# AER-RC/monoRTM

Hardware: AMD Instinct MI355X
Metric: (wavenumber x layer x line) optical-depth evals/sec (higher is better)
Workload: dtype f64; 1 GPU; c4: configs[3] whole: 1024 synthetic sonde profiles x 64 layers x 50 channels x 500 lines, f64, profile-sharded over 1 GPU(s): 1024 profiles on this rank; layers=64, wavenumbers=50, lines=500, nmol=7, launch=3 stream launches, parallelism=profile-sharded x1

## Files before the change

monortm_amd/_build.py:

```python
from __future__ import annotations

import os
import shutil
import subprocess

PKG = os.path.dirname(os.path.abspath(__file__))
ROOT = os.path.dirname(PKG)
CSRC = os.path.join(PKG, "csrc")
FSRC = os.path.join(PKG, "fortran")
LIBDIR = os.path.join(PKG, "lib")
LIB = os.path.join(LIBDIR, "libmonortm_hip.so")

HIPCC = os.environ.get("HIPCC", "/opt/rocm/bin/hipcc")
FC = os.environ.get("MONORTM_FC", "/opt/rocm/bin/amdflang")
HIP_SOURCES = ["api.hip", "lines_kernel.hip", "lines_ms_kernel.hip", "far_kernel.hip", "continuum_kernel.hip", "xsec_kernel.hip", "xsec_jac_kernel.hip", "rtm_kernel.hip", "rtm_scan_kernel.hip", "jacobian_kernel.hip", "rtm_scan_jac_kernel.hip", "rtm_obs_jac_kernel.hip", "rtm_obs_kernel.hip", "oe_kernel.hip", "line_table.cpp"]
HIP_DEPS = HIP_SOURCES + ["device_common.hpp", "lineshape.hpp", "cloud_tkc.hpp", "obs_exchange.hpp", "rtm_tile.hpp", "modm_plan.hpp", "ms_reach.hpp", "lines_device.hpp", "xsec_walk.hpp", "lines_asm.hpp", "lines_ms_asm.hpp", "line_table.hpp", "tables/monortm_tables.h",
                           "../../include/monortm_hip.h"]
HIP_FLAGS = ["--offload-arch=gfx950", "-O3", "-std=c++17", "-fPIC", "-shared", "-Wno-unused-value", "-Wno-pass-failed",
             "-Wno-unused-const-variable"]


_NO_LICM = ["-mllvm", "-disable-machine-licm"]
HIP_FILE_FLAGS = {"lines_ms_kernel.hip": _NO_LICM, "lines_kernel.hip": _NO_LICM, "continuum_kernel.hip": _NO_LICM, "rtm_obs_kernel.hip": _NO_LICM}


def _check_flags(flags: list[str]) -> None:
    extra = os.environ.get("MONORTM_EXTRA_HIPFLAGS", "").split()
    bad = [f for f in flags + extra if f.startswith(("-DFAR_ABL_", "-DMONORTM_ABLATE_", "-DMONORTM_NO_", "-DLINES_TIMING", "-DLINES_CLASS_STATS",
                                                     "-DMW_TIMING"))]
    if bad and os.environ.get("MONORTM_EXPERIMENT") != "1":
        raise RuntimeError(f"experiment switches in the build flags {bad}: set MONORTM_EXPERIMENT=1 (and use tools/build_variant.sh)")
# ... 82 lines not shown
```

monortm_amd/csrc/api.hip:

```cpp
#include <algorithm>
#include <atomic>
#include <chrono>
#include <cmath>
#include <cstdlib>
#include <cstdio>
#include <cstring>
#include <dlfcn.h>
#include <functional>
#include <initializer_list>
#include <string>
#include <vector>

#include "device_common.hpp"
#include "line_table.hpp"
#include "modm_plan.hpp"
#include "lineshape.hpp"
#include "tables/monortm_tables.h"

namespace {
using namespace monortm_dev;

thread_local std::string g_init_error;

struct Ctx {
    int device = 0;
    int cus = 256;
    size_t phys_cap = 2ull << 30, far_cap = 1ull << 30;
    std::vector<Ctx *> shards;
    struct Opt : ModmPlanOpt {
        int ms_ablate = 0;
        int ms_prepare = MS_PREPARE_FUSED;
        int ms_plan = 1;
        double jac_dt = MONORTM_JAC_DT, jac_dlnw = MONORTM_JAC_DLNW;
    } opt;
    void *comm = nullptr;
    int comm_rank = 0, comm_world = 1;
    bool has_lines = false;
    int real_kind = 8;
    std::string err;
    monortm::LineTable host;
    DevLines lines{};
    DevTables tables{};
    std::vector<void *> owned;
    int *errflag = nullptr;
    void *partial = nullptr;
    monortm_dev::MwCache mw_cache;
    void *phys = nullptr;
// ... 38 lines not shown
        const double *wpath = nullptr, *mw = nullptr;
        std::vector<int> shard;
    };
    static constexpr int kMaxObs = 16;
    Obs obs[kMaxObs];
    hipStream_t hs = nullptr;
    int *errflag_host = nullptr;
    struct {
        const void *dev = nullptr, *host = nullptr;
        size_t bytes = 0;
        int nprof = 0, nwn = 0, nlay_max = 0;
    } lastO;
    long long o_reused = 0;
    long long o_reused_scan = 0;
    long long finish_launches[6] = {0, 0, 0, 0, 0, 0};
    long long far_launches[4] = {0, 0, 0, 0};
    bool host_timing = false;
    double ht[3][4] = {{0, 0, 0, 0}, {0, 0, 0, 0}, {0, 0, 0, 0}};
    long long ht_calls[3] = {0, 0, 0};
    size_t partial_elems = 0;
    int profiling = 0;
    int prof_stride = 1;
    long long prof_calls[3] = {0, 0, 0};
    struct Ev {
        hipEvent_t a, b;
        int k;
    };
    std::vector<Ev> events;
    std::vector<hipEvent_t> event_pool;
    double tot_ms[3] = {0, 0, 0};
// ... 27 lines not shown
                           static_cast<const uint4 *>(src2), static_cast<uint4 *>(dst2), bytes2 / 16, flag_src, flag_dst);
        return hipGetLastError();
    }
    hipError_t e = hipMemcpyAsync(dst, src, bytes, kind, s);
    if (e == hipSuccess && flag_dst) e = hipMemcpyAsync(flag_dst, flag_src, sizeof(int), hipMemcpyDeviceToHost, s);
    if (e == hipSuccess && bytes2) e = hipMemcpyAsync(dst2, src2, bytes2, hipMemcpyDefault, s);
    return e;
}

void comm_release(Ctx *c);

int set_option(Ctx *c, const char *name, const char *value) {
    const std::string n = name ? name : "", v = value ? value : "";
    const bool autov = v.empty() || v == "auto";
    long iv = 0;
    double dv = 0.;
    bool isint = false, isdbl = false;
    if (!autov) {
        char *end = nullptr;
        iv = strtol(v.c_str(), &end, 10);
        isint = end && end != v.c_str() && *end == '\0';
        end = nullptr;
        dv = strtod(v.c_str(), &end);
        isdbl = end && end != v.c_str() && *end == '\0';
    }
    if (n == "nslice" && (autov || (isint && iv >= 1 && iv <= 16))) c->opt.nslice = autov ? 0 : (int)iv;
    else if (n == "fair" && (autov || (isint && (iv == 0 || iv == 1)))) c->opt.fair = autov ? -1 : (int)iv;
    else if (n == "tile_waves" && (autov || (isint && (iv == 1 || iv == 2 || iv == 4)))) c->opt.tile_waves = autov ? 0 : (int)iv;
    else if (n == "far_levels" && (autov || (isint && iv >= 0 && iv <= FAR_MAXLEV))) c->opt.far_levels = autov ? -1 : (int)iv;
    else if (n == "lines_kernel" && (autov || v == "wn" || v == "ms")) c->opt.lines_ms = autov ? -1 : (v == "ms" ? 1 : 0);
    else if (n == "ms_prepare" && (autov || v == "fused" || v == "passes")) c->opt.ms_prepare = v == "passes" ? MS_PREPARE_PASSES : MS_PREPARE_FUSED;
    else if (n == "ms_plan" && (autov || v == "on" || v == "off")) c->opt.ms_plan = v == "off" ? 0 : 1;
#ifdef MONORTM_EXPERIMENT
    else if (n == "ms_ablate" && isint && iv >= 0 && iv <= 9) c->opt.ms_ablate = (int)iv;
#endif
    else if (n == "finish" && (autov || v == "generic")) c->opt.finish_generic = autov ? 0 : 1;
    else if (n == "ms_items" && (autov || (isint && (iv == 64 || iv == 128 || iv == 192 || iv == 256)))) c->opt.ms_items = autov ? 0 : (int)iv;
    else if ((n == "jac_dt" || n == "jac_dlnw") && (autov || (isdbl && std::isfinite(dv) && dv > 0. && (n == "jac_dt" || dv < 1.)))) {
        if (n == "jac_dt") c->opt.jac_dt = autov ? MONORTM_JAC_DT : dv;
        else c->opt.jac_dlnw = autov ? MONORTM_JAC_DLNW : dv;
    }
    else { c->err = "unknown option or value: " + n + " = " + v; return MONORTM_EARG; }
    return MONORTM_OK;
}

template <class T>
int upload(Ctx *c, const T *src, size_t n, const T **dst) {
    void *p = nullptr;
    const size_t bytes = std::max<size_t>(n, 1) * sizeof(T);
    HIPCHK(c, hipMalloc(&p, bytes));
    c->owned.push_back(p);
// ... 802 lines not shown
        }
        if (hipGetLastError() != hipSuccess || hipDeviceSynchronize() != hipSuccess) { c->err = "log-ratio tables could not be formed"; return failed(MONORTM_EHIP); }
    }
    void *ef = nullptr;
    if (hipMalloc(&ef, sizeof(int)) != hipSuccess || hipMemset(ef, 0, sizeof(int)) != hipSuccess) { c->err = "hipMalloc(errflag) failed"; return failed(MONORTM_EHIP); }
    c->owned.push_back(ef);
    c->errflag = static_cast<int *>(ef);
    if (hipDeviceSynchronize() != hipSuccess) { c->err = "device set-up failed"; return failed(MONORTM_EHIP); }
    if (hipStreamCreateWithFlags(&c->hs, hipStreamNonBlocking) != hipSuccess ||
        hipHostMalloc(reinterpret_cast<void **>(&c->errflag_host), sizeof(int), hipHostMallocDefault) != hipSuccess) {
        c->err = "stream / pinned flag of the host-buffer entry points could not be created";
        return failed(MONORTM_EHIP);
    }
    if (const char *e = getenv("MONORTM_HOST_TIMING")) c->host_timing = e[0] == '1';
    if (getenv("MONORTM_FINISH_GENERIC")) c->opt.finish_generic = 1;
    for (const char *k : {"lines_kernel", "nslice", "fair", "tile_waves", "far_levels", "ms_items", "ms_prepare", "ms_plan",
#ifdef MONORTM_EXPERIMENT
                          "ms_ablate",
#endif
                         }) {
        std::string env = "MONORTM_" + std::string(k);
        for (char &ch : env) ch = (char)toupper((unsigned char)ch);
        if (const char *e = getenv(env.c_str()))
            if (set_option(c, k, e)) { c->err = env + ": " + c->err; return failed(MONORTM_EARG); }
    }
    if (c->host_timing && !g_timing_ctx) {
        g_timing_ctx = c;
        static bool registered = false;
        if (!registered) { atexit([] { if (g_timing_ctx) print_host_timing(g_timing_ctx); }); registered = true; }
    }
    *out = c;
// ... 252 lines not shown
    hipFree(din); hipFree(dtab); hipFree(dout);
    return rc ? rc : monortm_hip_check(c, nullptr);
}

long long monortm_hip_counter(void *ctx, int which) {
    Ctx *c = static_cast<Ctx *>(ctx);
    if (!c) return -1;
    if (!c->shards.empty()) {
        long long t = 0;
        for (Ctx *sh : c->shards) t += monortm_hip_counter(sh, which);
        return t;
    }
    if (which == 0) return c->o_reused;
    if (which == 1) return c->o_reused_scan;
    if (which >= 2 && which <= 7) return c->finish_launches[which - 2];
    if (which >= 16 && which <= 19) return c->far_launches[which - 16];
    return -1;
}

long long monortm_hip_line_count(void *ctx, int mol) {
    Ctx *c = static_cast<Ctx *>(ctx);
    if (!c || mol < 0 || mol > MXMOL) return -1;
    if (!c->shards.empty()) c = c->shards[0];
    return c->host.n_physical[mol];
}

int monortm_hip_profile(void *ctx, int enable) {
    Ctx *c = static_cast<Ctx *>(ctx);
    if (!c) return null_ctx();
    if (!c->shards.empty()) return multi_only_host(c);
// ... 184 lines not shown
        aw.nlay = a.nlay + pl.ms_nprof;
        aw.O = const_cast<void *>(shift(a.O, st * nwn)); aw.O_CLW = const_cast<void *>(shift(a.O_CLW, st * nwn));
        aw.O_BY_MOL = const_cast<void *>(shift(a.O_BY_MOL, st * nmol * nwn));
        aw.OC = const_cast<void *>(shift(a.OC, st * MONORTM_NCONT * nwn));
        aw.osum = a.osum ? a.osum + st * nwn : nullptr;
        launch_lines_ms(am, c->lines, c->tables, ms, pl.use_brd, s);
        launch_lines(aw, c->lines, c->tables, pl.nw, pl.wpl, pl.use_brd, dim3(grid.x, (unsigned)aw.nprof, grid.z), pl.dyn_lds, s);
    } else if (pl.use_ms) launch_lines_ms(a, c->lines, c->tables, ms, pl.use_brd, s);
    else launch_lines(a, c->lines, c->tables, pl.nw, pl.wpl, pl.use_brd, grid, pl.dyn_lds, s);
    prof_end(c, s, ev);
    HIPCHK(c, hipGetLastError());
    prof_begin(c, s, 1, ev);
    if (ixsect == 1 && !odx_given) launch_xsec(a, c->xs, s);
    a.slices_reduced = pl.slices_reduced;
    if (pl.slices_reduced) launch_reduce_slices(a, s);
    if (pl.mw) {
        const hipError_t e = launch_finish_mw(a, c->tables, vends[0], vends[1], pl.V1ABS, pl.V2ABS, pl.NPTABS, c->mw_cache, s);
        if (e != hipSuccess) {
            c->err = std::string("launch_finish_mw: ") + (c->mw_cache.why ? c->mw_cache.why : hipGetErrorString(e));
            return c->mw_cache.why ? MONORTM_EUNSUPPORTED : MONORTM_EHIP;
        }
    } else HIPCHK(c, launch_finish(a, c->tables, pl.V1ABS, pl.V2ABS, pl.NPTABS, pl.csize, pl.high, pl.par, pl.fin_threads, pl.fin_lds, pl.lds_sets, s));
    c->finish_launches[pl.finish_variant]++;
    prof_end(c, s, ev);
    HIPCHK(c, hipGetLastError());
    return MONORTM_OK;
}
}

extern "C" {

int monortm_hip_modm_xs_dev(void *ctx, int nprof, int nwn, const double *wn, double dvset, const int *nlay, int nlay_max,
                            int nmol, const void *P, const void *T, const void *CLW, const void *WKL,
                            const void *WBRODL, const double *cntnm_fac, double sclcpl, double sclhw, double y0res,
                            int ibrd, int ixsect, const void *XAMNT, void *ODXSEC, void *O, void *O_BY_MOL, void *OC,
                            void *O_CLW, const double *wn_ends, void *stream) {
    Ctx *c = static_cast<Ctx *>(ctx);
    if (!c) return null_ctx();
// ... 1168 lines not shown
```

monortm_amd/csrc/continuum_kernel.hip:

```cpp
#include "lineshape.hpp"
#include <cstring>
#include "cloud_tkc.hpp"
#include "tables/monortm_tables.h"

namespace {
using namespace monortm_dev;

struct AccGrid {
    double V1C, V2C, DVC;
    int NPTC, I1;
};
__host__ __device__ inline AccGrid acc_grid(double V1ABS, double V2ABS, double V1S, double DVS, int NPTS) {
    AccGrid g;
    g.DVC = DVS;
    g.V1C = V1ABS - g.DVC;
    g.V2C = V2ABS + g.DVC;
    if (g.V1C < V1S) g.I1 = -1;
    else g.I1 = (int)((g.V1C - V1S) / DVS + 0.01);
    g.V1C = V1S + DVS * (double)(g.I1 - 1);
    int I2 = (int)((g.V2C - V1S) / DVS + 0.01);
    g.NPTC = I2 - g.I1 + 3;
    if (g.NPTC > NPTS) g.NPTC = NPTS + 4;
    g.V2C = g.V1C + DVS * (double)(g.NPTC - 1);
    return g;
// ... 490 lines not shown
            const double VI = V1ABS + DVABS * (double)(I - 1);
            const double V1A = q.V1C[b], DVA = q.DVC[b], RECDVA = q.RDVC[b];
            const int J = (int)((VI - V1A) * RECDVA + K_ONEPL);
            const double VJ = V1A + DVA * (double)(J - 1);
            const double P = RECDVA * (VI - VJ);
            const double C = (3. - 2. * P) * P * P;
            const double B = 0.5 * P * (1. - P);
            const double B1 = B * (1. - P), B2 = B * P;
            r.B1 = B1, r.c1 = (1. - C + B2), r.c2 = (C + B1), r.B2 = B2;
            r.j = q.off[b] + J - 1;
            r.flags = b | 4;
        }
        ib[it] = r;
    }
}

template <typename R>
__global__ __launch_bounds__(256) __attribute__((amdgpu_waves_per_eu(8))) void finish_mw_kernel(ModmArgs a, MwSetup q, const MwItemA *__restrict__ ia, const MwItemB *__restrict__ ib,
                                                       double V1ABS, double V2ABS, int NPTABS) {
    extern __shared__ __attribute__((aligned(16))) double smem[];
    const int tid = threadIdx.x, nt = blockDim.x;
    const int lay = blockIdx.x, prof = blockIdx.y, iw0 = blockIdx.z * nt;
    const int nwn = a.nwn, nmol = a.nmol;
    const int iw = iw0 + tid;
    const size_t pl = (size_t)prof * a.nlay_max + lay;
#ifdef MW_TIMING
    long long tq[8]; int ntq = 0;
#define MW_T() tq[ntq++] = (long long)__builtin_readcyclecounter()
    MW_T();
#else
// ... 23 lines not shown
            for (int m = 0; m < nmol; m++) obm[(size_t)m * nwn + iw] = (R)0;
        }
        return;
    }
    if (sliced) {
        const int cw = min(nt, nwn - iw0);
        const size_t sstride = (size_t)a.nprof * a.nlay_max * nmol * nwn;
        const R *part = rp<R>(a.partial) + pl * nmol * (size_t)nwn;
        for (int it = tid; it < nmol * cw; it += nt) {
            const size_t at = (size_t)(it / cw) * nwn + iw0 + (it % cw);
            double acc = 0.;
            for (int sl = 0; sl < a.nslice; sl++) acc += (double)part[(size_t)sl * sstride + at];
            obm[at] = (R)acc;
        }
    }
    const double DVABS = 1.0;
    const double V1 = q.V1, V2 = q.V2;
    const double P0c = 1013., T0c = 296., XLOSMT = 2.68675E+19;
    const double rTAVE = rcp2(TAVE), rWTOT = rcp2(WTOT), pr = PAVE * (1. / P0c);
    const double RHOAVE = pr * (T0c * rTAVE);
    const double XKT = TAVE * (1. / K_RADCN2);
    const double amagat = pr * (273. * rTAVE);
    const double x_vmr_h2o = WK1 * rWTOT, x_vmr_o2 = WK7 * rWTOT, x_vmr_n2 = 1. - x_vmr_h2o - x_vmr_o2;
    const double wn2 = x_vmr_n2 * WTOT;
    const double h2o_fac = x_vmr_h2o;
    const double xself = a.cntnm[0], xfrgn = a.cntnm[1], xco2c = a.cntnm[2], xn2cn = a.cntnm[5];
    const bool on0 = q.alive[0] && xself > 0., on1 = q.alive[1] && xfrgn > 0., on2 = q.alive[2] && xco2c > 0.,
               on3 = q.alive[3] && xn2cn > 0.;
    double *sC = smem;
    double *sAbs = smem + q.off[4];
    const int NA = NPTABS + 4;

    MW_T();
    {
        const double Rself = h2o_fac * RHOAVE * 1.e-20 * xself;
        const double TFAC = (TAVE - T0c) * (1. / (260. - T0c));
        const double Rfrgn = (1. - h2o_fac) * RHOAVE * 1.e-20 * xfrgn;
        const double WCO2 = WK2 * RHOAVE * 1.0E-20 * xco2c;
        const double tau_fac = xn2cn * (wn2 / XLOSMT) * amagat;
        const double tfac = (TAVE - 296.) * (1. / (220. - 296.));
        const int onmask = (on0 ? 1 : 0) | (on1 ? 2 : 0) | (on2 ? 4 : 0) | (on3 ? 8 : 0);
        for (int it = tid; it < q.off[4]; it += nt) {
            const MwItemA r = ia[it];
            const int b = r.flags & 3;
            const bool live = ((r.flags >> 2) & 1) && ((onmask >> b) & 1), intab = (r.flags >> 3) & 1;
            const double ta = r.ta, tc = r.tc, te = r.te, tf = r.tf;
            const double pw1 = exp_cw((b == 0 ? TFAC : tfac) * ((b == 0 || b == 3) ? tc : 0.));
            const double pw2 = exp_cw(tfac * (b == 3 ? tf : 0.));
            double v = 0.;
            if (live) {
                if (b == 0) {
                    if (intab) {
                        double SH2O = 0.;
                        if (ta > 0.) SH2O = ta * pw1;
                        v = WK1 * (SH2O * Rself);
                    }
                } else if (b == 1) {
                    double FH2O = intab ? ta : 0.;
                    const double FSCAL = tc;
                    FH2O = FH2O * FSCAL;
                    v = (WK1 * FH2O) * Rfrgn;
                } else if (b == 2) {
                    if (intab) v = ta * WCO2;
                } else {
                    double c0 = 0., c1 = 0.;
                    if (intab) {
                        c0 = ta * pw1;
                        const double sf_T = te * pw2;
                        c1 = (sf_T - 1.) * (0.79) / (0.21);
                    }
                    v = tau_fac * c0 * (x_vmr_n2 + c1 * x_vmr_o2 + 1. * x_vmr_h2o);
                }
            }
            sC[it] = v;
        }
    }
    __syncthreads();

    MW_T();
    const int onmaskB = (on0 ? 1 : 0) | (on1 ? 2 : 0) | (on2 ? 4 : 0) | (on3 ? 8 : 0);
    for (int it = tid; it < 4 * NA; it += nt) {
        const MwItemB r = ib[it];
        const bool inside = ((r.flags >> 2) & 1) && ((onmaskB >> (r.flags & 3)) & 1);
        double v = 0.;
        if (inside) {
            const double *A = sC + r.j;
            v = (-A[0] * r.B1 + A[1] * r.c1 + A[2] * r.c2 - A[3] * r.B2) * 1.0;
        }
        sAbs[it] = v;
    }
    __syncthreads();

    MW_T();
    double soc = 0.;
    if (iw < nwn) {
        const double wnv = a.wn[iw];
        bool inside;
        double vint;
        if (a.dvset != 0.) {
            const int I = iw + 1;
            int ilo = (int)((V1ABS + DVABS - V1) / a.dvset + 1. + K_ONEMI);
            if (ilo < 1) ilo = 1;
            int ihi = (int)((V2ABS - DVABS - V1) / a.dvset + K_ONEMI);
            if (ihi > nwn) ihi = nwn;
            inside = I >= ilo && I <= ihi;
            vint = V1 + a.dvset * (double)(I - 1);
        } else {
            int ilo = (int)((V1ABS + DVABS - wnv) / 1.0 + 1. + K_ONEMI);
            if (ilo < 1) ilo = 1;
            int ihi = (int)((V2ABS - DVABS - wnv) / 1.0 + K_ONEMI);
            if (ihi > 1) ihi = 1;
            inside = ilo <= 1 && ihi >= 1;
            vint = wnv;
        }
        double rad = wnv;
        {
            const double x = (wnv * K_RADCN2) * rTAVE;
            if (x <= 0.01) rad = 0.5 * x * wnv;
            else if (x <= 10.0) {
                const double e = exp_cw(-x);
                rad = wnv * (1. - e) * rcp2(1. + e);
            }
        }
        const double RECDVA = 1. / DVABS;
        const int J = (int)((vint - V1ABS) * RECDVA + K_ONEPL);
        const double VJ = V1ABS + DVABS * (double)(J - 1);
        const double P = RECDVA * (vint - VJ);
        const double C = (3. - 2. * P) * P * P;
        const double B = 0.5 * P * (1. - P);
        const double B1 = B * (1. - P), B2 = B * P;
        double val[3] = {0., 0., 0.};
        if (inside) {
            const double *A0 = sAbs, *A1 = sAbs + NA, *A2 = sAbs + 2 * NA, *A3 = sAbs + 3 * NA;
            const double h0 = A0[J - 1] + A1[J - 1], h1 = A0[J] + A1[J], h2 = A0[J + 1] + A1[J + 1], h3 = A0[J + 2] + A1[J + 2];
            val[0] = -h0 * B1 + h1 * (1. - C + B2) + h2 * (C + B1) - h3 * B2;
            val[1] = -A2[J - 1] * B1 + A2[J] * (1. - C + B2) + A2[J + 1] * (C + B1) - A2[J + 2] * B2;
            val[2] = -A3[J - 1] * B1 + A3[J] * (1. - C + B2) + A3[J + 1] * (C + B1) - A3[J + 2] * B2;
        }
        const R s0 = (on0 || on1) ? (R)(val[0] * rad) : (R)0;
        const R s1 = on2 ? (R)(val[1] * rad) : (R)0;
        const R s4 = on3 ? (R)(val[2] * rad) : (R)0;
        OC[iw] = s0;
        OC[(size_t)nwn + iw] = s1;
        OC[(size_t)2 * nwn + iw] = (R)0;
        OC[(size_t)3 * nwn + iw] = (R)0;
        OC[(size_t)4 * nwn + iw] = s4;
        soc += (double)s0;
        soc += (double)s1;
        soc += 0.;
        soc += 0.;
        soc += (double)s4;
    }

    MW_T();
    if (iw < nwn) {
        if (sliced)
            for (int m = 0; m < nmol; m++) o_lines = o_lines + (double)obm[(size_t)m * nwn + iw];
        const double oclw = (CLW == 0.) ? 0. : odclw_tkc(a.wn[iw], TAVE, CLW);
        OCLW[iw] = (R)oclw;
        const double odx = a.ODXSEC ? (double)rp<R>(a.ODXSEC)[pl * (size_t)nwn + iw] : 0.;
        const double o = o_lines + odx + 0. + soc + oclw;
        O[iw] = (R)o;
    }
#ifdef LINES_TIMING
    if (a.osum && tid < 12 && blockIdx.z == 0) OCLW[8 + tid] = (R)a.osum[pl * (size_t)nwn + tid];
#endif
#ifdef MW_TIMING
    MW_T();
    if (tid == 0) for (int i = 1; i < ntq; i++) OCLW[i - 1] = (R)(double)(tq[i] - tq[i - 1]);
    if (tid == 0) OCLW[ntq - 1] = (R)(double)(tq[ntq - 1] - tq[0]);
#endif
}

template <typename R>
__global__ __launch_bounds__(256) void reduce_slices_kernel(ModmArgs a) {
    const int idx = blockIdx.x * 256 + threadIdx.x, lay = blockIdx.y, prof = blockIdx.z;
    const int n = a.nmol * a.nwn;
    if (idx >= n || lay >= a.nlay[prof]) return;
    const size_t pl = (size_t)prof * a.nlay_max + lay;
    const size_t sstride = (size_t)a.nprof * a.nlay_max * n;
    const R *part = rp<R>(a.partial) + pl * n;
    double acc = 0.;
    for (int sl = 0; sl < a.nslice; sl++) acc += (double)part[(size_t)sl * sstride + idx];
    wp<R>(a.O_BY_MOL)[pl * n + idx] = (R)acc;
}

// ... 22 lines not shown
    else if (which == 10) r0 = exp_cw(a[0]);
    else if (which == 11) r0 = rcp2(a[0]);
    out[2 * i] = r0;
    out[2 * i + 1] = r1;
}

}

namespace monortm_dev {
void launch_kat(int which, int n, const double *in, const double *tab, double *out, int *errflag, const DevTables &tb, hipStream_t s) {
    hipLaunchKernelGGL(kat_kernel, dim3((n + 63) / 64), dim3(64), 0, s, which, n, in, tab, out, errflag, tb);
}
void launch_logratio(const double *t296, const double *tlow, double *out, int n, hipStream_t s) {
    hipLaunchKernelGGL(logratio_kernel, dim3((n + 255) / 256), dim3(256), 0, s, t296, tlow, out, n);
}
hipError_t launch_finish_mw(const ModmArgs &a, const DevTables &tb, double V1, double V2, double V1ABS, double V2ABS, int NPTABS,
                            MwCache &cache, hipStream_t s) {
    MwSetup q;
    const double v1s[4] = {MT_SELF296_V1, MT_FRGN296_V1, MT_FCO2_V1, MT_N2RT296_V1};
    const double v2s[4] = {MT_SELF296_V2, MT_FRGN296_V2, MT_FCO2_V2, MT_N2RT296_V2};
    const double dvs[4] = {MT_SELF296_DV, MT_FRGN296_DV, MT_FCO2_DV, MT_N2RT296_DV};
    const int npt[4] = {MT_SELF296_NPT, MT_FRGN296_NPT, MT_FCO2_NPT, MT_N2RT296_NPT};
    const double DVABS = 1.0;
    q.off[0] = 0;
    for (int b = 0; b < 4; b++) {
        const AccGrid g = acc_grid(V1ABS, V2ABS, v1s[b], dvs[b], npt[b]);
        q.V1C[b] = g.V1C, q.DVC[b] = g.DVC, q.RDVC[b] = 1. / g.DVC, q.NPTC[b] = g.NPTC, q.I1[b] = g.I1, q.NPT[b] = npt[b];
        int ist = (int)(2 + (v1s[b] - V1ABS) / DVABS + 1.e-5);
        if (ist < 1) ist = 1;
        int last = (int)(1 + (v2s[b] - V1ABS) / DVABS + 1.e-5);
        if (last > NPTABS) last = NPTABS;
        q.ILO[b] = (int)((g.V1C + g.DVC - V1ABS) / DVABS + 1. + K_ONEMI);
// ... 54 lines not shown
        cache.e[cache.n] = ne;
        en = &cache.e[cache.n++];
    } else if (!en->ready) {
        hipStreamCaptureStatus cap = hipStreamCaptureStatusNone;
        (void)hipStreamIsCapturing(s, &cap);
        if (cap == hipStreamCaptureStatusNone && hipEventQuery(en->built) == hipSuccess) en->ready = true;
        else {
            (void)hipGetLastError();
            hipError_t e = hipStreamWaitEvent(s, en->built, 0);
            if (e != hipSuccess) return e;
        }
    }
    en->last_use = ++cache.clock;
    const MwItemA *ia = static_cast<const MwItemA *>(en->items);
    const MwItemB *ib = reinterpret_cast<const MwItemB *>(ia + nA);
    if (a.real_kind == 4) hipLaunchKernelGGL(finish_mw_kernel<float>, grid, dim3(threads), lds, s, a, q, ia, ib, V1ABS, V2ABS, NPTABS);
    else hipLaunchKernelGGL(finish_mw_kernel<double>, grid, dim3(threads), lds, s, a, q, ia, ib, V1ABS, V2ABS, NPTABS);
    return hipGetLastError();
}
void MwCache::release() {
    for (int i = 0; i < n; i++) {
        (void)hipFree(e[i].items);
        (void)hipEventDestroy(e[i].built);
    }
    n = 0;
}
void launch_reduce_slices(const ModmArgs &a, hipStream_t s) {
    const dim3 grid((a.nmol * a.nwn + 255) / 256, a.nlay_max, a.nprof);
    if (a.real_kind == 4) hipLaunchKernelGGL(reduce_slices_kernel<float>, grid, dim3(256), 0, s, a);
    else hipLaunchKernelGGL(reduce_slices_kernel<double>, grid, dim3(256), 0, s, a);
// ... 28 lines not shown
```

monortm_amd/csrc/device_common.hpp:

```cpp
#pragma once
#include <hip/hip_runtime.h>

#if (defined(FAR_ABL_HOT) || defined(FAR_ABL_STEPS) || defined(FAR_ABL_TRANS) || defined(MONORTM_ABLATE_LOOP) || defined(MONORTM_ABLATE_EVAL) || \
     defined(MONORTM_ABLATE_VOIGT) || defined(MONORTM_ABLATE_ZSEARCH) || defined(MONORTM_ABLATE_EXP4) || defined(MONORTM_ABLATE_COUPLE) ||     \
     defined(MONORTM_NO_CLAMP_GUARD) || defined(MONORTM_NO_UNIFIED) || defined(MONORTM_NO_VSCAN) ||              \
     defined(MONORTM_NO_HALF) || defined(MONORTM_NO_FULL) || defined(MONORTM_NO_CHUNKFAR) || defined(MONORTM_NO_SGL_TSKIP) || defined(LINES_TIMING) || \
     defined(LINES_CLASS_STATS) || defined(MW_TIMING)) &&                                                                                          \
    !defined(MONORTM_EXPERIMENT)
#error "a timing-experiment / A-B switch of monortm_amd is defined: such builds are measurements, not the product - add -DMONORTM_EXPERIMENT=1"
#endif

#include <cstdint>

#include "../../include/monortm_hip.h"

namespace monortm_dev {

#define K_PI 3.1415926535898
#define K_PLANCK 6.62606876E-27
#define K_BOLTZ 1.3806503E-16
#define K_CLIGHT 2.99792458E+10
#define K_AVOGAD 6.02214199E+23
#define K_RADCN1 1.191042722E-12
#define K_RADCN2 1.4387752
// ... 336 lines not shown
        double key[5];
        void *items;
        hipEvent_t built;
        hipStream_t stream;
        bool ready;
        unsigned long long last_use;
    };
    static constexpr int kMax = 8;
    Entry e[kMax];
    int n = 0;
    unsigned long long clock = 0;
    const char *why = nullptr;
    void release();
};
hipError_t launch_finish_mw(const ModmArgs &a, const DevTables &tb, double V1, double V2, double V1ABS, double V2ABS, int NPTABS, MwCache &cache,
                            hipStream_t s);
void launch_kat(int which, int n, const double *in, const double *tab, double *out, int *errflag, const DevTables &tb, hipStream_t s);
void launch_xsec(const ModmArgs &a, const DevXsec &x, hipStream_t s);
void launch_xsec_jac(const XsecJacArgs &a, const DevXsec &x, hipStream_t s);
void launch_rtm(const RtmArgs &a, hipStream_t s);
void launch_rtm_scan(const RtmScanArgs &a, hipStream_t s);
void launch_jac_perturb(const JacPerturbArgs &a, hipStream_t s);
void launch_rtm_jac(const RtmJacArgs &a, bool full, hipStream_t s);
void launch_rtm_scan_jac(const RtmScanJacArgs &a, bool full, hipStream_t s);
void launch_rtm_obs_jac(const RtmObsJacArgs &a, bool full, int out_kind, hipStream_t s);
void launch_rtm_obs(const RtmObsArgs &a, int out_kind, hipStream_t s);
hipError_t launch_oe_step(const OeArgs &a, hipStream_t s);
hipError_t launch_oe_cov(const OeCovArgs &a, hipStream_t s);

}
```

Measured before the change: 1714 billion evals/s.

## Add column-layout finish_mw kernel processing 64 layers per workgroup

Adds a new microwave-continuum finish kernel in which each workgroup handles up to 64 layers of one profile. Phase-A coefficients are computed per layer into a strided LDS column, and then each wave walks its layers to interpolate and write optical depths, prefetching the next layer's line and xsec values. The per-layer setup code is factored into shared helpers, and an auto heuristic picks the column path when there are at most 64 wavenumbers, enough layers and enough workgroups. The aim is to amortise the item-table reads and the per-layer launch granularity, at the cost of higher LDS use and per-wave serial loops.

```diff
diff --git a/monortm_amd/_build.py b/monortm_amd/_build.py
--- a/monortm_amd/_build.py
+++ b/monortm_amd/_build.py
@@ -14,7 +14,7 @@
 HIPCC = os.environ.get("HIPCC", "/opt/rocm/bin/hipcc")
 FC = os.environ.get("MONORTM_FC", "/opt/rocm/bin/amdflang")
 HIP_SOURCES = ["api.hip", "lines_kernel.hip", "lines_ms_kernel.hip", "far_kernel.hip", "continuum_kernel.hip", "xsec_kernel.hip", "xsec_jac_kernel.hip", "rtm_kernel.hip", "rtm_scan_kernel.hip", "jacobian_kernel.hip", "rtm_scan_jac_kernel.hip", "rtm_obs_jac_kernel.hip", "rtm_obs_kernel.hip", "oe_kernel.hip", "line_table.cpp"]
-HIP_DEPS = HIP_SOURCES + ["device_common.hpp", "lineshape.hpp", "cloud_tkc.hpp", "obs_exchange.hpp", "rtm_tile.hpp", "modm_plan.hpp", "ms_reach.hpp", "lines_device.hpp", "xsec_walk.hpp", "lines_asm.hpp", "lines_ms_asm.hpp", "line_table.hpp", "tables/monortm_tables.h",
+HIP_DEPS = HIP_SOURCES + ["device_common.hpp", "lineshape.hpp", "cloud_tkc.hpp", "obs_exchange.hpp", "rtm_tile.hpp", "modm_plan.hpp", "finish_mw_layout.hpp", "ms_reach.hpp", "lines_device.hpp", "xsec_walk.hpp", "lines_asm.hpp", "lines_ms_asm.hpp", "line_table.hpp", "tables/monortm_tables.h",
                            "../../include/monortm_hip.h"]
 HIP_FLAGS = ["--offload-arch=gfx950", "-O3", "-std=c++17", "-fPIC", "-shared", "-Wno-unused-value", "-Wno-pass-failed",
              "-Wno-unused-const-variable"]
diff --git a/monortm_amd/csrc/api.hip b/monortm_amd/csrc/api.hip
--- a/monortm_amd/csrc/api.hip
+++ b/monortm_amd/csrc/api.hip
@@ -14,6 +14,7 @@
 #include "device_common.hpp"
 #include "line_table.hpp"
 #include "modm_plan.hpp"
+#include "finish_mw_layout.hpp"
 #include "lineshape.hpp"
 #include "tables/monortm_tables.h"
 
@@ -31,6 +32,7 @@
         int ms_ablate = 0;
         int ms_prepare = MS_PREPARE_FUSED;
         int ms_plan = 1;
+        int finish_mw = monortm_dev::FINISH_MW_AUTO;
         double jac_dt = MONORTM_JAC_DT, jac_dlnw = MONORTM_JAC_DLNW;
     } opt;
     void *comm = nullptr;
@@ -99,6 +101,7 @@
     long long o_reused = 0;
     long long o_reused_scan = 0;
     long long finish_launches[6] = {0, 0, 0, 0, 0, 0};
+    long long finish_mw_col_launches = 0;
     long long far_launches[4] = {0, 0, 0, 0};
     bool host_timing = false;
     double ht[3][4] = {{0, 0, 0, 0}, {0, 0, 0, 0}, {0, 0, 0, 0}};
@@ -156,6 +159,7 @@
     const std::string n = name ? name : "", v = value ? value : "";
     const bool autov = v.empty() || v == "auto";
     long iv = 0;
+    int iopt = 0;
     double dv = 0.;
     bool isint = false, isdbl = false;
     if (!autov) {
@@ -177,6 +181,7 @@
     else if (n == "ms_ablate" && isint && iv >= 0 && iv <= 9) c->opt.ms_ablate = (int)iv;
 #endif
     else if (n == "finish" && (autov || v == "generic")) c->opt.finish_generic = autov ? 0 : 1;
+    else if (n == "finish_mw" && monortm_dev::finish_mw_parse(v.c_str(), &iopt)) c->opt.finish_mw = iopt;
     else if (n == "ms_items" && (autov || (isint && (iv == 64 || iv == 128 || iv == 192 || iv == 256)))) c->opt.ms_items = autov ? 0 : (int)iv;
     else if ((n == "jac_dt" || n == "jac_dlnw") && (autov || (isdbl && std::isfinite(dv) && dv > 0. && (n == "jac_dt" || dv < 1.)))) {
         if (n == "jac_dt") c->opt.jac_dt = autov ? MONORTM_JAC_DT : dv;
@@ -1009,7 +1014,7 @@
     }
     if (const char *e = getenv("MONORTM_HOST_TIMING")) c->host_timing = e[0] == '1';
     if (getenv("MONORTM_FINISH_GENERIC")) c->opt.finish_generic = 1;
-    for (const char *k : {"lines_kernel", "nslice", "fair", "tile_waves", "far_levels", "ms_items", "ms_prepare", "ms_plan",
+    for (const char *k : {"lines_kernel", "nslice", "fair", "tile_waves", "far_levels", "ms_items", "ms_prepare", "ms_plan", "finish_mw",
 #ifdef MONORTM_EXPERIMENT
                           "ms_ablate",
 #endif
@@ -1292,6 +1297,7 @@
     if (which == 0) return c->o_reused;
     if (which == 1) return c->o_reused_scan;
     if (which >= 2 && which <= 7) return c->finish_launches[which - 2];
+    if (which == 9) return c->finish_mw_col_launches;
     if (which >= 16 && which <= 19) return c->far_launches[which - 16];
     return -1;
 }
@@ -1506,14 +1512,16 @@
     if (ixsect == 1 && !odx_given) launch_xsec(a, c->xs, s);
     a.slices_reduced = pl.slices_reduced;
     if (pl.slices_reduced) launch_reduce_slices(a, s);
+    bool column = false;
     if (pl.mw) {
-        const hipError_t e = launch_finish_mw(a, c->tables, vends[0], vends[1], pl.V1ABS, pl.V2ABS, pl.NPTABS, c->mw_cache, s);
+        const hipError_t e = launch_finish_mw(a, c->tables, vends[0], vends[1], pl.V1ABS, pl.V2ABS, pl.NPTABS, c->mw_cache, c->opt.finish_mw, c->cus, &column, s);
         if (e != hipSuccess) {
             c->err = std::string("launch_finish_mw: ") + (c->mw_cache.why ? c->mw_cache.why : hipGetErrorString(e));
             return c->mw_cache.why ? MONORTM_EUNSUPPORTED : MONORTM_EHIP;
         }
     } else HIPCHK(c, launch_finish(a, c->tables, pl.V1ABS, pl.V2ABS, pl.NPTABS, pl.csize, pl.high, pl.par, pl.fin_threads, pl.fin_lds, pl.lds_sets, s));
     c->finish_launches[pl.finish_variant]++;
+    if (column) c->finish_mw_col_launches++;
     prof_end(c, s, ev);
     HIPCHK(c, hipGetLastError());
     return MONORTM_OK;
diff --git a/monortm_amd/csrc/continuum_kernel.hip b/monortm_amd/csrc/continuum_kernel.hip
--- a/monortm_amd/csrc/continuum_kernel.hip
+++ b/monortm_amd/csrc/continuum_kernel.hip
@@ -2,6 +2,7 @@
 #include <cstring>
 #include "cloud_tkc.hpp"
 #include "tables/monortm_tables.h"
+#include "finish_mw_layout.hpp"
 
 namespace {
 using namespace monortm_dev;
@@ -528,6 +529,137 @@
         ib[it] = r;
     }
 }
+
+struct MwLayer {
+    double TAVE, rTAVE, WK1, x_vmr_h2o, x_vmr_o2, x_vmr_n2;
+    double Rself, TFAC, Rfrgn, WCO2, tau_fac, tfac;
+};
+__device__ __forceinline__ MwLayer mw_layer(double PAVE, double TAVE, double WTOT, double WK1, double WK2, double WK7, double xself,
+                                            double xfrgn, double xco2c, double xn2cn) {
+    const double P0c = 1013., T0c = 296., XLOSMT = 2.68675E+19;
+    MwLayer L;
+    const double rTAVE = rcp2(TAVE), rWTOT = rcp2(WTOT), pr = PAVE * (1. / P0c);
+    const double RHOAVE = pr * (T0c * rTAVE);
+    const double amagat = pr * (273. * rTAVE);
+    const double x_vmr_h2o = WK1 * rWTOT, x_vmr_o2 = WK7 * rWTOT, x_vmr_n2 = 1. - x_vmr_h2o - x_vmr_o2;
+    const double wn2 = x_vmr_n2 * WTOT;
+    const double h2o_fac = x_vmr_h2o;
+    L.TAVE = TAVE, L.rTAVE = rTAVE, L.WK1 = WK1, L.x_vmr_h2o = x_vmr_h2o, L.x_vmr_o2 = x_vmr_o2, L.x_vmr_n2 = x_vmr_n2;
+    L.Rself = h2o_fac * RHOAVE * 1.e-20 * xself;
+    L.TFAC = (TAVE - T0c) * (1. / (260. - T0c));
+    L.Rfrgn = (1. - h2o_fac) * RHOAVE * 1.e-20 * xfrgn;
+    L.WCO2 = WK2 * RHOAVE * 1.0E-20 * xco2c;
+    L.tau_fac = xn2cn * (wn2 / XLOSMT) * amagat;
+    L.tfac = (TAVE - 296.) * (1. / (220. - 296.));
+    return L;
+}
+__device__ __forceinline__ double mw_a_self(const MwLayer &L, double ta, double pw1, bool intab) {
+    double v = 0.;
+    if (intab) {
+        double SH2O = 0.;
+        if (ta > 0.) SH2O = ta * pw1;
+        v = L.WK1 * (SH2O * L.Rself);
+    }
+    return v;
+}
+__device__ __forceinline__ double mw_a_frgn(const MwLayer &L, double ta, double tc, bool intab) {
+    double FH2O = intab ? ta : 0.;
+    const double FSCAL = tc;
+    FH2O = FH2O * FSCAL;
+    return (L.WK1 * FH2O) * L.Rfrgn;
+}
+__device__ __forceinline__ double mw_a_co2(const MwLayer &L, double ta, bool intab) {
+    return intab ? ta * L.WCO2 : 0.;
+}
+__device__ __forceinline__ double mw_a_n2(const MwLayer &L, double ta, double te, double pw1, double pw2, bool intab) {
+    double c0 = 0., c1 = 0.;
+    if (intab) {
+        c0 = ta * pw1;
+        const double sf_T = te * pw2;
+        c1 = (sf_T - 1.) * (0.79) / (0.21);
+    }
+    return L.tau_fac * c0 * (L.x_vmr_n2 + c1 * L.x_vmr_o2 + 1. * L.x_vmr_h2o);
+}
+__device__ __forceinline__ double mw_b_point(double a0, double a1, double a2, double a3, const MwItemB &r) {
+    return (-a0 * r.B1 + a1 * r.c1 + a2 * r.c2 - a3 * r.B2) * 1.0;
+}
+struct MwChan {
+    double wnv, B1, w1, w2, B2;
+    int J;
+    bool inside;
+};
+__device__ __forceinline__ MwChan mw_chan(const ModmArgs &a, double V1, double V1ABS, double V2ABS, int iw) {
+    const double DVABS = 1.0;
+    const int nwn = a.nwn;
+    MwChan c;
+    const double wnv = a.wn[iw];
+    double vint;
+    if (a.dvset != 0.) {
+        const int I = iw + 1;
+        int ilo = (int)((V1ABS + DVABS - V1) / a.dvset + 1. + K_ONEMI);
+        if (ilo < 1) ilo = 1;
+        int ihi = (int)((V2ABS - DVABS - V1) / a.dvset + K_ONEMI);
+        if (ihi > nwn) ihi = nwn;
+        c.inside = I >= ilo && I <= ihi;
+        vint = V1 + a.dvset * (double)(I - 1);
+    } else {
+        int ilo = (int)((V1ABS + DVABS - wnv) / 1.0 + 1. + K_ONEMI);
+        if (ilo < 1) ilo = 1;
+        int ihi = (int)((V2ABS - DVABS - wnv) / 1.0 + K_ONEMI);
+        if (ihi > 1) ihi = 1;
+        c.inside = ilo <= 1 && ihi >= 1;
+        vint = wnv;
+    }
+    const double RECDVA = 1. / DVABS;
+    const int J = (int)((vint - V1ABS) * RECDVA + K_ONEPL);
+    const double VJ = V1ABS + DVABS * (double)(J - 1);
+    const double P = RECDVA * (vint - VJ);
+    const double tP = (3. - 2. * P) * P;
+    const double B = 0.5 * P * (1. - P);
+    const double B1 = B * (1. - P), B2 = B * P;
+    c.wnv = wnv, c.J = J, c.B1 = B1, c.w1 = fma(B, P, fma(-tP, P, 1.)), c.w2 = fma(tP, P, B1), c.B2 = B2;
+    return c;
+}
+__device__ __forceinline__ double mw_radfn(double wnv, double rTAVE) {
+    double rad = wnv;
+    const double x = (wnv * K_RADCN2) * rTAVE;
+    if (x <= 0.01) rad = 0.5 * x * wnv;
+    else if (x <= 10.0) {
+        const double e = exp_cw(-x);
+        rad = wnv * (1. - e) * rcp2(1. + e);
+    }
+    return rad;
+}
+__device__ __forceinline__ void mw_xint3(const double *sAbs, int NA, const MwChan &c, double val[3]) {
+    val[0] = val[1] = val[2] = 0.;
+    if (c.inside) {
+        const int J = c.J;
+        const double *A0 = sAbs, *A1 = sAbs + NA, *A2 = sAbs + 2 * NA, *A3 = sAbs + 3 * NA;
+        const double h0 = A0[J - 1] + A1[J - 1], h1 = A0[J] + A1[J], h2 = A0[J + 1] + A1[J + 1], h3 = A0[J + 2] + A1[J + 2];
+        val[0] = -h0 * c.B1 + h1 * c.w1 + h2 * c.w2 - h3 * c.B2;
+        val[1] = -A2[J - 1] * c.B1 + A2[J] * c.w1 + A2[J + 1] * c.w2 - A2[J + 2] * c.B2;
+        val[2] = -A3[J - 1] * c.B1 + A3[J] * c.w1 + A3[J + 1] * c.w2 - A3[J + 2] * c.B2;
+    }
+}
+template <typename R>
+__device__ __forceinline__ double mw_store_oc(R *OC, size_t nwn, int iw, const double val[3], double rad, bool on01, bool on2, bool on3) {
+    const R s0 = on01 ? (R)(val[0] * rad) : (R)0;
+    const R s1 = on2 ? (R)(val[1] * rad) : (R)0;
+    const R s4 = on3 ? (R)(val[2] * rad) : (R)0;
+    OC[iw] = s0;
+    OC[nwn + iw] = s1;
+    OC[2 * nwn + iw] = (R)0;
+    OC[3 * nwn + iw] = (R)0;
+    OC[4 * nwn + iw] = s4;
+    double soc = 0.;
+    soc += (double)s0;
+    soc += (double)s1;
+    soc += 0.;
+    soc += 0.;
+    soc += (double)s4;
+    return soc;
+}
+__device__ __forceinline__ double mw_total(double o_lines, double odx, double soc, double oclw) { return o_lines + odx + 0. + soc + oclw; }
 
 template <typename R>
 __global__ __launch_bounds__(256) __attribute__((amdgpu_waves_per_eu(8))) void finish_mw_kernel(ModmArgs a, MwSetup q, const MwItemA *__restrict__ ia, const MwItemB *__restrict__ ib,
@@ -581,17 +713,9 @@
             obm[at] = (R)acc;
         }
     }
-    const double DVABS = 1.0;
-    const double V1 = q.V1, V2 = q.V2;
-    const double P0c = 1013., T0c = 296., XLOSMT = 2.68675E+19;
-    const double rTAVE = rcp2(TAVE), rWTOT = rcp2(WTOT), pr = PAVE * (1. / P0c);
-    const double RHOAVE = pr * (T0c * rTAVE);
-    const double XKT = TAVE * (1. / K_RADCN2);
-    const double amagat = pr * (273. * rTAVE);
-    const double x_vmr_h2o = WK1 * rWTOT, x_vmr_o2 = WK7 * rWTOT, x_vmr_n2 = 1. - x_vmr_h2o - x_vmr_o2;
-    const double wn2 = x_vmr_n2 * WTOT;
-    const double h2o_fac = x_vmr_h2o;
+    const double V1 = q.V1;
     const double xself = a.cntnm[0], xfrgn = a.cntnm[1], xco2c = a.cntnm[2], xn2cn = a.cntnm[5];
+    const MwLayer L = mw_layer(PAVE, TAVE, WTOT, WK1, WK2, WK7, xself, xfrgn, xco2c, xn2cn);
     const bool on0 = q.alive[0] && xself > 0., on1 = q.alive[1] && xfrgn > 0., on2 = q.alive[2] && xco2c > 0.,
                on3 = q.alive[3] && xn2cn > 0.;
     double *sC = smem;
@@ -600,44 +724,20 @@
 
     MW_T();
     {
-        const double Rself = h2o_fac * RHOAVE * 1.e-20 * xself;
-        const double TFAC = (TAVE - T0c) * (1. / (260. - T0c));
-        const double Rfrgn = (1. - h2o_fac) * RHOAVE * 1.e-20 * xfrgn;
-        const double WCO2 = WK2 * RHOAVE * 1.0E-20 * xco2c;
-        const double tau_fac = xn2cn * (wn2 / XLOSMT) * amagat;
-        const double tfac = (TAVE - 296.) * (1. / (220. - 296.));
         const int onmask = (on0 ? 1 : 0) | (on1 ? 2 : 0) | (on2 ? 4 : 0) | (on3 ? 8 : 0);
         for (int it = tid; it < q.off[4]; it += nt) {
             const MwItemA r = ia[it];
             const int b = r.flags & 3;
             const bool live = ((r.flags >> 2) & 1) && ((onmask >> b) & 1), intab = (r.flags >> 3) & 1;
             const double ta = r.ta, tc = r.tc, te = r.te, tf = r.tf;
-            const double pw1 = exp_cw((b == 0 ? TFAC : tfac) * ((b == 0 || b == 3) ? tc : 0.));
-            const double pw2 = exp_cw(tfac * (b == 3 ? tf : 0.));
+            const double pw1 = exp_cw((b == 0 ? L.TFAC : L.tfac) * ((b == 0 || b == 3) ? tc : 0.));
+            const double pw2 = exp_cw(L.tfac * (b == 3 ? tf : 0.));
             double v = 0.;
             if (live) {
-                if (b == 0) {
-                    if (intab) {
-                        double SH2O = 0.;
-                        if (ta > 0.) SH2O = ta * pw1;
-                        v = WK1 * (SH2O * Rself);
-                    }
-                } else if (b == 1) {
-                    double FH2O = intab ? ta : 0.;
-                    const double FSCAL = tc;
-                    FH2O = FH2O * FSCAL;
-                    v = (WK1 * FH2O) * Rfrgn;
-                } else if (b == 2) {
-                    if (intab) v = ta * WCO2;
-                } else {
-                    double c0 = 0., c1 = 0.;
-                    if (intab) {
-                        c0 = ta * pw1;
-                        const double sf_T = te * pw2;
-                        c1 = (sf_T - 1.) * (0.79) / (0.21);
-                    }
-                    v = tau_fac * c0 * (x_vmr_n2 + c1 * x_vmr_o2 + 1. * x_vmr_h2o);
-                }
+                if (b == 0) v = mw_a_self(L, ta, pw1, intab);
+                else if (b == 1) v = mw_a_frgn(L, ta, tc, intab);
+                else if (b == 2) v = mw_a_co2(L, ta, intab);
+                else v = mw_a_n2(L, ta, te, pw1, pw2, intab);
             }
             sC[it] = v;
         }
@@ -652,7 +752,7 @@
         double v = 0.;
         if (inside) {
             const double *A = sC + r.j;
-            v = (-A[0] * r.B1 + A[1] * r.c1 + A[2] * r.c2 - A[3] * r.B2) * 1.0;
+            v = mw_b_point(A[0], A[1], A[2], A[3], r);
         }
         sAbs[it] = v;
     }
@@ -661,62 +761,11 @@
     MW_T();
     double soc = 0.;
     if (iw < nwn) {
-        const double wnv = a.wn[iw];
-        bool inside;
-        double vint;
-        if (a.dvset != 0.) {
-            const int I = iw + 1;
-            int ilo = (int)((V1ABS + DVABS - V1) / a.dvset + 1. + K_ONEMI);
-            if (ilo < 1) ilo = 1;
-            int ihi = (int)((V2ABS - DVABS - V1) / a.dvset + K_ONEMI);
-            if (ihi > nwn) ihi = nwn;
-            inside = I >= ilo && I <= ihi;
-            vint = V1 + a.dvset * (double)(I - 1);
-        } else {
-            int ilo = (int)((V1ABS + DVABS - wnv) / 1.0 + 1. + K_ONEMI);
-            if (ilo < 1) ilo = 1;
-            int ihi = (int)((V2ABS - DVABS - wnv) / 1.0 + K_ONEMI);
-            if (ihi > 1) ihi = 1;
-            inside = ilo <= 1 && ihi >= 1;
-            vint = wnv;
-        }
-        double rad = wnv;
-        {
-            const double x = (wnv * K_RADCN2) * rTAVE;
-            if (x <= 0.01) rad = 0.5 * x * wnv;
-            else if (x <= 10.0) {
-                const double e = exp_cw(-x);
-                rad = wnv * (1. - e) * rcp2(1. + e);
-            }
-        }
-        const double RECDVA = 1. / DVABS;
-        const int J = (int)((vint - V1ABS) * RECDVA + K_ONEPL);
-        const double VJ = V1ABS + DVABS * (double)(J - 1);
-        const double P = RECDVA * (vint - VJ);
-        const double C = (3. - 2. * P) * P * P;
-        const double B = 0.5 * P * (1. - P);
-        const double B1 = B * (1. - P), B2 = B * P;
-        double val[3] = {0., 0., 0.};
-        if (inside) {
-            const double *A0 = sAbs, *A1 = sAbs + NA, *A2 = sAbs + 2 * NA, *A3 = sAbs + 3 * NA;
-            const double h0 = A0[J - 1] + A1[J - 1], h1 = A0[J] + A1[J], h2 = A0[J + 1] + A1[J + 1], h3 = A0[J + 2] + A1[J + 2];
-            val[0] = -h0 * B1 + h1 * (1. - C + B2) + h2 * (C + B1) - h3 * B2;
-            val[1] = -A2[J - 1] * B1 + A2[J] * (1. - C + B2) + A2[J + 1] * (C + B1) - A2[J + 2] * B2;
-            val[2] = -A3[J - 1] * B1 + A3[J] * (1. - C + B2) + A3[J + 1] * (C + B1) - A3[J + 2] * B2;
-        }
-        const R s0 = (on0 || on1) ? (R)(val[0] * rad) : (R)0;
-        const R s1 = on2 ? (R)(val[1] * rad) : (R)0;
-        const R s4 = on3 ? (R)(val[2] * rad) : (R)0;
-        OC[iw] = s0;
-        OC[(size_t)nwn + iw] = s1;
-        OC[(size_t)2 * nwn + iw] = (R)0;
-        OC[(size_t)3 * nwn + iw] = (R)0;
-        OC[(size_t)4 * nwn + iw] = s4;
-        soc += (double)s0;
-        soc += (double)s1;
-        soc += 0.;
-        soc += 0.;
-        soc += (double)s4;
+        const MwChan c = mw_chan(a, V1, V1ABS, V2ABS, iw);
+        const double rad = mw_radfn(c.wnv, L.rTAVE);
+        double val[3];
+        mw_xint3(sAbs, NA, c, val);
+        soc = mw_store_oc<R>(OC, (size_t)nwn, iw, val, rad, on0 || on1, on2, on3);
     }
 
     MW_T();
@@ -726,8 +775,7 @@
         const double oclw = (CLW == 0.) ? 0. : odclw_tkc(a.wn[iw], TAVE, CLW);
         OCLW[iw] = (R)oclw;
         const double odx = a.ODXSEC ? (double)rp<R>(a.ODXSEC)[pl * (size_t)nwn + iw] : 0.;
-        const double o = o_lines + odx + 0. + soc + oclw;
-        O[iw] = (R)o;
+        O[iw] = (R)mw_total(o_lines, odx, soc, oclw);
     }
 #ifdef LINES_TIMING
     if (a.osum && tid < 12 && blockIdx.z == 0) OCLW[8 + tid] = (R)a.osum[pl * (size_t)nwn + tid];
@@ -737,6 +785,167 @@
     if (tid == 0) for (int i = 1; i < ntq; i++) OCLW[i - 1] = (R)(double)(tq[i] - tq[i - 1]);
     if (tid == 0) OCLW[ntq - 1] = (R)(double)(tq[ntq - 1] - tq[0]);
 #endif
+}
+
+__device__ __forceinline__ double mw_readlane(double x, int l) {
+    const int lo = __builtin_amdgcn_readlane(__double2loint(x), l), hi = __builtin_amdgcn_readlane(__double2hiint(x), l);
+    return __hiloint2double(hi, lo);
+}
+__device__ __forceinline__ double mw_opaque(double x) {
+    asm volatile("" : "+v"(x));
+    return x;
+}
+template <typename R>
+__device__ __forceinline__ void mw_col_point(const ModmArgs &a, const MwChan &c, const double *sAbs, int NA, double rTAVE, double TAVE,
+                                             double CLW, bool on01, bool on2, bool on3, double o_lines, double odx, size_t pl, int iw) {
+    const size_t nwn = (size_t)a.nwn;
+    const double wnv = mw_opaque(c.wnv);
+    const double rad = mw_radfn(wnv, rTAVE);
+    double val[3];
+    mw_xint3(sAbs, NA, c, val);
+    const double soc = mw_store_oc<R>(wp<R>(a.OC) + pl * MONORTM_NCONT * nwn, nwn, iw, val, rad, on01, on2, on3);
+    const double oclw = (CLW == 0.) ? 0. : odclw_tkc(wnv, TAVE, CLW);
+    wp<R>(a.O_CLW)[pl * nwn + iw] = (R)oclw;
+    wp<R>(a.O)[pl * nwn + iw] = (R)mw_total(o_lines, odx, soc, oclw);
+}
+template <typename R>
+__device__ __forceinline__ double mw_col_lines(const ModmArgs &a, size_t pl, int iw) {
+    const size_t nwn = (size_t)a.nwn;
+    if (a.osum) return a.osum[pl * nwn + iw];
+    double o_lines = 0.;
+    const R *obm = rp<R>(a.O_BY_MOL) + pl * a.nmol * nwn;
+    for (int m = 0; m < a.nmol; m++) o_lines = o_lines + (double)obm[(size_t)m * nwn + iw];
+    return o_lines;
+}
+template <typename R>
+__device__ __forceinline__ double mw_col_odx(const ModmArgs &a, size_t pl, int iw) {
+    return a.ODXSEC ? (double)rp<R>(a.ODXSEC)[pl * (size_t)a.nwn + iw] : 0.;
+}
+
+template <typename R, int NW, bool MULTI>
+__global__ __launch_bounds__(NW * 64) void finish_mw_kernel_col(ModmArgs a, MwSetup q, const MwItemA *__restrict__ ia, const MwItemB *__restrict__ ib,
+                                                                double V1ABS, double V2ABS, int NPTABS) {
+    extern __shared__ __attribute__((aligned(16))) double smem[];
+    constexpr int KB = 3;
+    const int lane = threadIdx.x & 63, wave = __builtin_amdgcn_readfirstlane((int)(threadIdx.x >> 6));
+    const int prof = blockIdx.y, lay0 = blockIdx.x * 64;
+    const int nwn = a.nwn, nmol = a.nmol;
+    const int nblk = min(64, a.nlay_max - lay0);
+    const int nact = max(0, min(nblk, a.nlay[prof] - lay0));
+    const size_t pl0 = (size_t)prof * a.nlay_max + lay0;
+    const int nA = q.off[4], NA = NPTABS + 4, nB = 4 * NA;
+    double *sC = smem;
+    double *sAbs = smem + (size_t)nA * MW_COL_STRIDE + (size_t)wave * nB;
+
+    {
+        const int per = (nblk - nact + NW - 1) / NW;
+        const int z0 = min(nblk, nact + wave * per), z1 = min(nblk, z0 + per);
+        for (int l = z0; l < z1; l++) {
+            const size_t pl = pl0 + l;
+            R *O = wp<R>(a.O) + pl * (size_t)nwn, *OCLW = wp<R>(a.O_CLW) + pl * (size_t)nwn;
+            R *OC = wp<R>(a.OC) + pl * MONORTM_NCONT * (size_t)nwn, *obm = wp<R>(a.O_BY_MOL) + pl * nmol * (size_t)nwn;
+            for (int iw = lane; iw < nwn; iw += 64) {
+                O[iw] = (R)0;
+                OCLW[iw] = (R)0;
+                for (int sl = 0; sl < MONORTM_NCONT; sl++) OC[(size_t)sl * nwn + iw] = (R)0;
+                for (int m = 0; m < nmol; m++) obm[(size_t)m * nwn + iw] = (R)0;
+            }
+        }
+    }
+    if (nact == 0) return;
+
+    const double xself = a.cntnm[0], xfrgn = a.cntnm[1], xco2c = a.cntnm[2], xn2cn = a.cntnm[5];
+    const bool on0 = q.alive[0] && xself > 0., on1 = q.alive[1] && xfrgn > 0., on2 = q.alive[2] && xco2c > 0.,
+               on3 = q.alive[3] && xn2cn > 0.;
+    const int onmask = (on0 ? 1 : 0) | (on1 ? 2 : 0) | (on2 ? 4 : 0) | (on3 ? 8 : 0);
+    double TAVE, CLW, rTAVE;
+    {
+        const size_t pl = pl0 + min(lane, nact - 1);
+        const double PAVE = rp<R>(a.P)[pl], WBROAD = rp<R>(a.WBRODL)[pl];
+        TAVE = rp<R>(a.T)[pl], CLW = rp<R>(a.CLW)[pl];
+        const R *wk = rp<R>(a.WKL) + pl * nmol;
+        double WTOT = WBROAD;
+        for (int m = 0; m < nmol; m++) WTOT = WTOT + wk[m];
+        const double WK1 = wk[0], WK2 = wk[1], WK7 = wk[6];
+        const MwLayer L = mw_layer(PAVE, TAVE, WTOT, WK1, WK2, WK7, xself, xfrgn, xco2c, xn2cn);
+        rTAVE = L.rTAVE;
+        for (int it = wave; it < nA; it += NW) {
+            const MwItemA r = ia[it];
+            const int b = r.flags & 3;
+            const bool live = ((r.flags >> 2) & 1) && ((onmask >> b) & 1), intab = (r.flags >> 3) & 1;
+            double v = 0.;
+            if (live) {
+                if (b == 0) v = mw_a_self(L, r.ta, exp_cw(L.TFAC * r.tc), intab);
+                else if (b == 1) v = mw_a_frgn(L, r.ta, r.tc, intab);
+                else if (b == 2) v = mw_a_co2(L, r.ta, intab);
+                else v = mw_a_n2(L, r.ta, r.te, exp_cw(L.tfac * r.tc), exp_cw(L.tfac * r.tf), intab);
+            }
+            sC[it * MW_COL_STRIDE + lane] = v;
+        }
+    }
+    __syncthreads();
+
+    const int per = (nact + NW - 1) / NW;
+    const int la0 = min(nact, wave * per), la1 = min(nact, la0 + per);
+    if (la0 >= la1) return;
+    MwItemB rb[KB];
+    bool inB[KB];
+#pragma unroll
+    for (int k = 0; k < KB; k++) {
+        const int it = lane + 64 * k;
+        rb[k] = MwItemB{0., 0., 0., 0., 0, 0};
+        if (it < nB) rb[k] = ib[it];
+        inB[k] = ((rb[k].flags >> 2) & 1) && ((onmask >> (rb[k].flags & 3)) & 1);
+    }
+    const double V1 = q.V1;
+    const int ncb = MULTI ? (nwn + 63) / 64 : 1;
+    MwChan c0{};
+    double pre_o = 0., pre_x = 0.;
+    if (!MULTI && lane < nwn) {
+        c0 = mw_chan(a, V1, V1ABS, V2ABS, lane);
+        pre_o = mw_col_lines<R>(a, pl0 + la0, lane), pre_x = mw_col_odx<R>(a, pl0 + la0, lane);
+    }
+    for (int l = la0; l < la1; l++) {
+        const size_t pl = pl0 + l;
+        const double rT = mw_readlane(rTAVE, l), T = mw_readlane(TAVE, l), W = mw_readlane(CLW, l);
+        const double cur_o = pre_o, cur_x = pre_x;
+        if (!MULTI && lane < nwn && l + 1 < la1) pre_o = mw_col_lines<R>(a, pl + 1, lane), pre_x = mw_col_odx<R>(a, pl + 1, lane);
+        const double *col = sC + l;
+#pragma unroll
+        for (int k = 0; k < KB; k++) {
+            const int it = lane + 64 * k;
+            if (it < nB) {
+                double v = 0.;
+                if (inB[k]) {
+                    const double *A = col + rb[k].j * MW_COL_STRIDE;
+                    v = mw_b_point(A[0], A[MW_COL_STRIDE], A[2 * MW_COL_STRIDE], A[3 * MW_COL_STRIDE], rb[k]);
+                }
+                sAbs[it] = v;
+            }
+        }
+        for (int it = lane + 64 * KB; it < nB; it += 64) {
+            const MwItemB r = ib[it];
+            double v = 0.;
+            if (((r.flags >> 2) & 1) && ((onmask >> (r.flags & 3)) & 1)) {
+                const double *A = col + r.j * MW_COL_STRIDE;
+                v = mw_b_point(A[0], A[MW_COL_STRIDE], A[2 * MW_COL_STRIDE], A[3 * MW_COL_STRIDE], r);
+            }
+            sAbs[it] = v;
+        }
+        team_sync<false>();
+        if (!MULTI) {
+            if (lane < nwn) mw_col_point<R>(a, c0, sAbs, NA, rT, T, W, on0 || on1, on2, on3, cur_o, cur_x, pl, lane);
+        } else {
+            for (int cb = 0; cb < ncb; cb++) {
+                const int iw = cb * 64 + lane;
+                if (iw < nwn) {
+                    const MwChan c = mw_chan(a, V1, V1ABS, V2ABS, iw);
+                    mw_col_point<R>(a, c, sAbs, NA, rT, T, W, on0 || on1, on2, on3, mw_col_lines<R>(a, pl, iw), mw_col_odx<R>(a, pl, iw), pl, iw);
+                }
+            }
+        }
+        team_sync<false>();
+    }
 }
 
 template <typename R>
@@ -789,8 +998,14 @@
 void launch_logratio(const double *t296, const double *tlow, double *out, int n, hipStream_t s) {
     hipLaunchKernelGGL(logratio_kernel, dim3((n + 255) / 256), dim3(256), 0, s, t296, tlow, out, n);
 }
+template <typename R, int NW>
+static void launch_finish_mw_col(bool multi, dim3 grid, size_t lds, hipStream_t s, const ModmArgs &a, const MwSetup &q, const MwItemA *ia,
+                                 const MwItemB *ib, double V1ABS, double V2ABS, int NPTABS) {
+    if (multi) hipLaunchKernelGGL((finish_mw_kernel_col<R, NW, true>), grid, dim3(NW * 64), lds, s, a, q, ia, ib, V1ABS, V2ABS, NPTABS);
+    else hipLaunchKernelGGL((finish_mw_kernel_col<R, NW, false>), grid, dim3(NW * 64), lds, s, a, q, ia, ib, V1ABS, V2ABS, NPTABS);
+}
 hipError_t launch_finish_mw(const ModmArgs &a, const DevTables &tb, double V1, double V2, double V1ABS, double V2ABS, int NPTABS,
-                            MwCache &cache, hipStream_t s) {
+                            MwCache &cache, int layout_opt, int cus, bool *column, hipStream_t s) {
     MwSetup q;
     const double v1s[4] = {MT_SELF296_V1, MT_FRGN296_V1, MT_FCO2_V1, MT_N2RT296_V1};
     const double v2s[4] = {MT_SELF296_V2, MT_FRGN296_V2, MT_FCO2_V2, MT_N2RT296_V2};
@@ -875,6 +1090,18 @@
     en->last_use = ++cache.clock;
     const MwItemA *ia = static_cast<const MwItemA *>(en->items);
     const MwItemB *ib = reinterpret_cast<const MwItemB *>(ia + nA);
+    int col_nw = finish_mw_col_waves(MwLayoutIn{a.nprof, a.nlay_max, a.nwn, cus, nA, NPTABS, sliced, layout_opt});
+#if defined(LINES_TIMING) || defined(MW_TIMING)
+    col_nw = 0;
+#endif
+    if (column) *column = col_nw != 0;
+    if (col_nw) {
+        const dim3 cgrid((a.nlay_max + 63) / 64, a.nprof);
+        const size_t clds = finish_mw_col_lds(nA, NPTABS, col_nw);
+        if (a.real_kind == 4) launch_finish_mw_col<float, 4>(a.nwn > 64, cgrid, clds, s, a, q, ia, ib, V1ABS, V2ABS, NPTABS);
+        else launch_finish_mw_col<double, 4>(a.nwn > 64, cgrid, clds, s, a, q, ia, ib, V1ABS, V2ABS, NPTABS);
+        return hipGetLastError();
+    }
     if (a.real_kind == 4) hipLaunchKernelGGL(finish_mw_kernel<float>, grid, dim3(threads), lds, s, a, q, ia, ib, V1ABS, V2ABS, NPTABS);
     else hipLaunchKernelGGL(finish_mw_kernel<double>, grid, dim3(threads), lds, s, a, q, ia, ib, V1ABS, V2ABS, NPTABS);
     return hipGetLastError();
diff --git a/monortm_amd/csrc/device_common.hpp b/monortm_amd/csrc/device_common.hpp
--- a/monortm_amd/csrc/device_common.hpp
+++ b/monortm_amd/csrc/device_common.hpp
@@ -374,7 +374,7 @@
     void release();
 };
 hipError_t launch_finish_mw(const ModmArgs &a, const DevTables &tb, double V1, double V2, double V1ABS, double V2ABS, int NPTABS, MwCache &cache,
-                            hipStream_t s);
+                            int layout_opt, int cus, bool *column, hipStream_t s);
 void launch_kat(int which, int n, const double *in, const double *tab, double *out, int *errflag, const DevTables &tb, hipStream_t s);
 void launch_xsec(const ModmArgs &a, const DevXsec &x, hipStream_t s);
 void launch_xsec_jac(const XsecJacArgs &a, const DevXsec &x, hipStream_t s);
diff --git a/monortm_amd/csrc/finish_mw_layout.hpp b/monortm_amd/csrc/finish_mw_layout.hpp
--- /dev/null
+++ b/monortm_amd/csrc/finish_mw_layout.hpp
@@ -0,0 +1,41 @@
+#pragma once
+#include <cstddef>
+#include <cstring>
+
+namespace monortm_dev {
+
+enum { FINISH_MW_AUTO = 0, FINISH_MW_LAYER = 1, FINISH_MW_COLUMN = 2 };
+
+inline bool finish_mw_parse(const char *v, int *out) {
+    if (!v || !*v || !strcmp(v, "auto")) *out = FINISH_MW_AUTO;
+    else if (!strcmp(v, "layer")) *out = FINISH_MW_LAYER;
+    else if (!strcmp(v, "column")) *out = FINISH_MW_COLUMN;
+    else return false;
+    return true;
+}
+
+constexpr int MW_COL_STRIDE = 65;
+constexpr size_t MW_COL_LDS_MAX = 40960;
+
+inline size_t finish_mw_col_lds(int nA, int NPTABS, int nw) {
+    return sizeof(double) * ((size_t)nA * MW_COL_STRIDE + (size_t)nw * 4 * (size_t)(NPTABS + 4));
+}
+
+struct MwLayoutIn {
+    int nprof, nlay_max, nwn, cus;
+    int nA, NPTABS;
+    bool sliced;
+    int opt;
+};
+
+inline int finish_mw_col_waves(const MwLayoutIn &in) {
+    const int nw = 4;
+    if (in.opt == FINISH_MW_LAYER || in.sliced) return 0;
+    if (finish_mw_col_lds(in.nA, in.NPTABS, nw) > MW_COL_LDS_MAX) return 0;
+    if (in.opt == FINISH_MW_COLUMN) return nw;
+    const long long wgs = (long long)in.nprof * ((in.nlay_max + 63) / 64);
+    if (in.nwn > 64 || in.nlay_max < 32 || wgs < 4ll * in.cus) return 0;
+    return nw;
+}
+
+}
```

Measured after the change: 1760 billion evals/s, median of 6. 2.7% higher.
